# sina-behnam/RTSDS

Hardware: AMD Instinct MI355X
Metric: images/sec/node (train step) + inference FPS@1024x512, BiSeNet 19-cls (higher is better)
Workload: dtype bf16; 1 GPU; configs[1]: BiSeNet-R18 seg-only train step (train.py:65-113); model=BiSeNet-ResNet18, global_batch=8, per_gpu_batch=8, image=3x512x1024, num_classes=19, parallelism=dp1

## Files before the change

### include/rtsds_hip.h

```cpp
#ifndef RTSDS_HIP_H
#define RTSDS_HIP_H
#include <stddef.h>
#include <stdint.h>
#ifdef __cplusplus
extern "C" {
#endif

enum { RTSDS_F32 = 0, RTSDS_BF16 = 1, RTSDS_F16 = 2  };
enum {
  RTSDS_OK = 0,
  RTSDS_ERR_SHAPE = 1,
  RTSDS_ERR_UNSUPPORTED = 2,
  RTSDS_ERR_LAUNCH = 3,
  RTSDS_ERR_WORKSPACE = 4
};
enum { RTSDS_ACT_NONE = 0, RTSDS_ACT_RELU = 1, RTSDS_ACT_LEAKY = 2, RTSDS_ACT_SIGMOID = 3 };
#define RTSDS_ACCUMULATE 0x100
#define RTSDS_INPUT_PADDED 0x400
#define RTSDS_WEIGHT_PACKED 0x800

typedef struct {
  int n, h, w, c;
  int ho, wo, k;
  int kh, kw;
// ... 39 lines not shown
  int nv;
  int cv, cp;
  int splits, accumulate;
} rtsds_split_reduce_desc;
int rtsds_conv2d_wgrad_deferred(const rtsds_conv_desc* d, const void* x, const void* dy, float* dw,
                                float* dbias, int accumulate, void* ws, size_t ws_bytes,
                                rtsds_split_reduce_desc* pending, void* stream);
int rtsds_split_reduce_many(int n, const rtsds_split_reduce_desc* descs, void* stream);
size_t rtsds_imgconv_bn_wgrad_workspace(const rtsds_conv_desc* d);
int rtsds_imgconv_bn_wgrad(const rtsds_conv_desc* d, const void* x, const void* bn_dy, const void* bn_x,
                           const float* coef, int act, float* dw, int accumulate, void* ws, size_t ws_bytes,
                           void* stream);
int rtsds_imgconv_bn_wgrad_deferred(const rtsds_conv_desc* d, const void* x, const void* bn_dy, const void* bn_x,
                                    const float* coef, int act, float* dw, int accumulate, void* ws,
                                    size_t ws_bytes, rtsds_split_reduce_desc* pending, void* stream);

size_t rtsds_bn_workspace(long rows, int c);
int rtsds_bn_fwd(const void* x, const void* res, void* y, long rows, int c, const float* gamma,
                 const float* beta, float* running_mean, float* running_var,
                 long long* num_batches_tracked, float* save_mean,
                 float* save_invstd, float momentum, float eps, int training, int act,
                 const float* stats_part, int stats_nrb, int dtype, void* ws, size_t ws_bytes,
                 void* stream);
int rtsds_bn_fwd_ld(const void* x, const void* res, void* y, long ldy, long rows, int c,
                    const float* gamma, const float* beta, float* running_mean, float* running_var,
                    long long* num_batches_tracked, float* save_mean, float* save_invstd,
                    float momentum, float eps, int training, int act, const float* stats_part,
                    int stats_nrb, int dtype, void* ws, size_t ws_bytes, void* stream);
int rtsds_bn_fold(const float* gamma, const float* beta, const float* running_mean,
                  const float* running_var, const float* conv_bias, float eps, int c, float* scale,
// ... 268 lines not shown
                        void* pooled, void* hid, void* att, void* r, int ldr, int n, long hw, int c, int dtype,
                        void* stream);
int rtsds_ffm_att_bwd(const void* dr, const void* f, const void* a, const void* h, const void* p, const void* w1,
                      const void* w2, float* dw1, float* db1, float* dw2, float* db2, void* dp, int n, long hw, int c,
                      int accumulate, int dtype, void* ws, size_t ws_bytes, void* stream);
int rtsds_bn_bwd_ffm(const void* dr, const void* att, const void* dpooled, int n, long hw, const void* x, void* dx,
                     float* dgamma, float* dbeta, int c, const float* gamma, const float* beta, const float* save_mean,
                     const float* save_invstd, int training, int act, int accumulate_params, int dtype, void* ws,
                     size_t ws_bytes, void* stream);

size_t rtsds_label_stats_workspace(int n, int c);
int rtsds_label_stats(const int64_t* label, int n, int h, int w, int c, int ignore_index,
                      unsigned long long* count, unsigned long long* support, void* ws, size_t ws_bytes,
                      void* stream);

#define RTSDS_ABI_VERSION 27
int rtsds_abi_version(void);

#ifdef __cplusplus
}
#endif
#endif
```

### rtsds_amd/_lib.py

```python
import ctypes
import os

import torch

_HERE = os.path.dirname(os.path.abspath(__file__))
DEFAULT_LIB_PATH = os.path.join(_HERE, "librtsds_hip.so")
ABI_VERSION = 27
LIB_PATH = os.environ.get("RTSDS_LIB") or DEFAULT_LIB_PATH

F32, BF16 = 0, 1
ACT_NONE, ACT_RELU, ACT_LEAKY, ACT_SIGMOID = 0, 1, 2, 3
ACCUMULATE = 0x100
INPUT_PADDED = 0x400
WEIGHT_PACKED = 0x800
UPCE_SET_CORRECT = 2
ERRORS = {1: "bad shape", 2: "unsupported configuration", 3: "HIP launch failure", 4: "workspace too small"}

c_int, c_long, c_float, c_double, c_size_t, c_void_p = (ctypes.c_int, ctypes.c_long, ctypes.c_float, ctypes.c_double,
                                                        ctypes.c_size_t, ctypes.c_void_p)


class ConvDesc(ctypes.Structure):
    _fields_ = [(n, c_int) for n in ("n", "h", "w", "c", "ho", "wo", "k", "kh", "kw", "sh", "sw",
                                     "ph", "pw", "dh", "dw", "dtype")]


class SplitReduceDesc(ctypes.Structure):
    _fields_ = [("slab", c_void_p), ("dw", c_void_p), ("slab_stride", c_long), ("nv", c_int), ("cv", c_int),
                ("cp", c_int), ("splits", c_int), ("accumulate", c_int)]


class BnParams(ctypes.Structure):
    _fields_ = [("gamma", c_void_p), ("beta", c_void_p), ("running_mean", c_void_p), ("running_var", c_void_p),
                ("num_batches_tracked", c_void_p), ("save_mean", c_void_p), ("save_invstd", c_void_p),
                ("momentum", c_float), ("eps", c_float), ("stats_part", c_void_p), ("stats_nrb", c_int),
                ("accumulate", c_int), ("dgamma", c_void_p), ("dbeta", c_void_p)]


P = c_void_p
SIGNATURES = {
    "rtsds_conv2d_fwd_workspace": (c_size_t, [ctypes.POINTER(ConvDesc)]),
    "rtsds_conv2d_input_pitch": (c_int, [ctypes.POINTER(ConvDesc)]),
    "rtsds_conv2d_fwd_stats_tiles": (c_int, [ctypes.POINTER(ConvDesc)]),
    "rtsds_conv2d_fwd": (c_int, [ctypes.POINTER(ConvDesc), P, P, P, P, c_int, P, P, c_size_t, P]),
# ... 5 lines not shown
    "rtsds_conv2d_dgrad_pack_bytes": (c_size_t, [ctypes.POINTER(ConvDesc)]),
    "rtsds_conv2d_dgrad_pack_many": (c_int, [c_int, ctypes.POINTER(ConvDesc), P, P, P]),
    "rtsds_conv2d_dgrad": (c_int, [ctypes.POINTER(ConvDesc), P, P, P, c_int, P, c_size_t, P]),
    "rtsds_conv2d_dgrad_act": (c_int, [ctypes.POINTER(ConvDesc), P, P, P, P, c_int, P, c_size_t, P]),
    "rtsds_conv2d_dgrad_bnstats_tiles": (c_int, [ctypes.POINTER(ConvDesc)]),
    "rtsds_conv2d_dgrad_bnstats": (c_int, [ctypes.POINTER(ConvDesc), P, P, P, P, P, P, P, P, c_int, P, P, c_size_t, P]),
    "rtsds_conv2d_wgrad_workspace": (c_size_t, [ctypes.POINTER(ConvDesc)]),
    "rtsds_conv2d_wgrad": (c_int, [ctypes.POINTER(ConvDesc), P, P, P, P, c_int, P, c_size_t, P]),
    "rtsds_conv2d_wgrad_deferred": (c_int, [ctypes.POINTER(ConvDesc), P, P, P, P, c_int, P, c_size_t,
                                            ctypes.POINTER(SplitReduceDesc), P]),
    "rtsds_split_reduce_many": (c_int, [c_int, ctypes.POINTER(SplitReduceDesc), P]),
    "rtsds_imgconv_bn_wgrad_workspace": (c_size_t, [ctypes.POINTER(ConvDesc)]),
    "rtsds_imgconv_bn_wgrad": (c_int, [ctypes.POINTER(ConvDesc), P, P, P, P, c_int, P, c_int, P, c_size_t, P]),
    "rtsds_imgconv_bn_wgrad_deferred": (c_int, [ctypes.POINTER(ConvDesc), P, P, P, P, c_int, P, c_int, P, c_size_t,
                                                ctypes.POINTER(SplitReduceDesc), P]),
    "rtsds_bn_workspace": (c_size_t, [c_long, c_int]),
    "rtsds_bn_bwd_coef": (c_int, [P, P, P, P, P, c_long, c_int, P, P, P, P, c_int, c_int, c_int, c_int, P, c_size_t, P]),
    "rtsds_bn_fwd": (c_int, [P, P, P, c_long, c_int, P, P, P, P, P, P, P, c_float, c_float, c_int,
                             c_int, P, c_int, c_int, P, c_size_t, P]),
    "rtsds_bn_fwd_ld": (c_int, [P, P, P, c_long, c_long, c_int, P, P, P, P, P, P, P, c_float, c_float, c_int,
                                c_int, P, c_int, c_int, P, c_size_t, P]),
    "rtsds_bn_fold": (c_int, [P, P, P, P, P, c_float, c_int, P, P, P]),
    "rtsds_pooled_mlp_fwd": (c_int, [P, P, P, P, P, P, P, c_int, c_int, c_int, c_int, c_int, P]),
    "rtsds_pooled_mlp_bwd": (c_int, [P, P, P, P, P, P, P, P, P, P, P, c_int, c_int, c_int, c_int, c_int, c_int, P]),
    "rtsds_bn_fwd_gap": (c_int, [P, P, P, c_int, c_long, c_int, P, P, P, P, P, P, P, c_float, c_float, c_int, P, c_int,
                                 c_int, P, c_size_t, P]),
    "rtsds_ffm_att_scale": (c_int, [P] * 10 + [c_int, c_int, c_long, c_int, c_int, P]),
    "rtsds_ffm_att_bwd": (c_int, [P] * 12 + [c_int, c_long, c_int, c_int, c_int, P, c_size_t, P]),
    "rtsds_bn_bwd_ffm": (c_int, [P, P, P, c_int, c_long, P, P, P, P, c_int, P, P, P, P, c_int, c_int, c_int, c_int,
                                 P, c_size_t, P]),
# ... 161 lines not shown
```

### rtsds_amd/csrc/bn.hip

```cpp
#include "bn_dev.h"
#include "chan_dev.h"
#include <type_traits>
#include <algorithm>

static const int kBnMaxRB = 2048;
static const int kBnTinyRows = 64;

template <int VEC> struct BnLayout {
  int tpr, rpi;
  __host__ __device__ BnLayout(int c) {
    tpr = (c + VEC - 1) / VEC;
    if (tpr > 256) tpr = 256;
    rpi = 256 / tpr;
  }
};
template <int VEC> struct BnTile : BnLayout<VEC> {
  int cl, cv, rg, ch0, cvalid;
  bool col, active;
  RT_DEV static int block_channels(int c) { return min(c - (int)blockIdx.y * 256 * VEC, 256 * VEC); }
  RT_DEV BnTile(int c) : BnLayout<VEC>(block_channels(c)) {
    cl = block_channels(c);
    cv = threadIdx.x % this->tpr;
    rg = threadIdx.x / this->tpr;
    ch0 = blockIdx.y * 256 * VEC + cv * VEC;
    cvalid = c - ch0;
    col = cv * VEC < cl;
    active = rg < this->rpi && col;
  }
  RT_DEV long row0() const { return (long)blockIdx.x * this->rpi + rg; }
  RT_DEV long step() const { return (long)gridDim.x * this->rpi; }
};

RT_DEV void bn_coef(float g, float b, float m, float inv, float& sc, float& sh) {
  sc = g * inv;
  sh = fmaf(-m, sc, b);
}

RT_DEV void chan_merge(float& na, float& ma, float& Ma, float nb, float mb, float Mb) {
  if (nb == 0.f) return;
  if (na == 0.f) { na = nb; ma = mb; Ma = Mb; return; }
  const float n = na + nb, d = mb - ma;
  ma += d * (nb / n);
  Ma += Mb + d * d * (na * nb / n);
  na = n;
}

template <typename T, int VEC>
__global__ void __launch_bounds__(256) bn_stats_kernel(const T* __restrict__ x, float* __restrict__ part, long rows, int c) {
  __shared__ float sh[3][256][VEC];
  const BnTile<VEC> t(c);
  const int tid = threadIdx.x, ch0 = t.ch0;
// ... 436 lines not shown
  __syncthreads();
  if (t.rg != 0 || !t.col) return false;
#pragma unroll
  for (int j = 0; j < VEC; ++j) {
    float a = red[0][tid][j], b = red[1][tid][j];
    for (int gi = 1; gi < t.rpi; ++gi) {
      a += red[0][gi * t.tpr + t.cv][j];
      b += red[1][gi * t.tpr + t.cv][j];
    }
    sg[j] = a;
    sgx[j] = b;
  }
  return true;
}

struct BnBwdOps {
  float inv = 0.f, g = 1.f, bt = 0.f, mu = 0.f, dg0 = 0.f, db0 = 0.f;
};
RT_DEV BnBwdOps bn_bwd_ops(int ch, const float* gamma, const float* beta, const float* smean, const float* sinv,
                           const float* dgamma, const float* dbeta, int accumulate) {
  BnBwdOps o;
  o.inv = sinv[ch];
  o.mu = smean[ch];
  if (gamma) o.g = gamma[ch];
  if (beta) o.bt = beta[ch];
  if (accumulate && dgamma) o.dg0 = dgamma[ch];
  if (accumulate && dbeta) o.db0 = dbeta[ch];
  return o;
}
RT_DEV void bn_bwd_tail(const BnBwdOps& o, float sg, float sgx, int ch, long rows, int training, int accumulate,
                        float* dgamma, float* dbeta, float& A, float& B, float& C) {
  const float inv = o.inv;
  if (dgamma) dgamma[ch] = accumulate ? o.dg0 + sgx * inv : sgx * inv;
  if (dbeta) dbeta[ch] = accumulate ? o.db0 + sg : sg;
  const float a = o.g * inv;
  const float invn = 1.f / (float)rows;
  A = a;
  B = training ? -a * inv * inv * sgx * invn : 0.f;
  C = training ? -a * sg * invn : 0.f;
}
RT_DEV void bn_bwd_coef_rows(const BnBwdOps& o, float sg, float sgx, int ch, int c, long rows, int training, int accumulate,
                             float* dgamma, float* dbeta, float* coef) {
  bn_bwd_tail(o, sg, sgx, ch, rows, training, accumulate, dgamma, dbeta, coef[ch], coef[c + ch], coef[2 * c + ch]);
  coef[3 * c + ch] = o.mu;
  bn_coef(o.g, o.bt, o.mu, o.inv, coef[4 * c + ch], coef[5 * c + ch]);
}

template <typename T, int VEC>
RT_DEV void bn_bwd_row_store(T* __restrict__ dx, T* __restrict__ dres, long off, const BnDx<VEC>& k, int cvalid, const float* g,
                             float* xv) {
#pragma unroll
  for (int j = 0; j < VEC; ++j) xv[j] = bn_bwd_dx<VEC>(k, j, g[j], xv[j]);
  if (dx) store_vec<T, VEC>(dx + off, xv, cvalid);
  if (dres) store_vec<T, VEC>(dres + off, g, cvalid);
}
// ... 872 lines not shown
```

### rtsds_amd/csrc/bn_dev.h

```cpp
#pragma once
#include "common.h"

template <typename T, int VEC>
RT_DEV void load_vec(const T* p, float* v, int cvalid) {
  static_assert(VEC == 1 || VEC == VecT<T>::N, "VEC");
  if constexpr (VEC == VecT<T>::N) {
    typename VecT<T>::v16 t = *(const typename VecT<T>::v16*)p;
#pragma unroll
    for (int j = 0; j < VEC; ++j) v[j] = to_f(t[j]);
  } else {
    v[0] = cvalid > 0 ? to_f(p[0]) : 0.f;
  }
}
template <typename T, int VEC>
RT_DEV void store_vec(T* p, const float* v, int cvalid) {
  if constexpr (VEC == VecT<T>::N) {
    typename VecT<T>::v16 t;
#pragma unroll
    for (int j = 0; j < VEC; ++j) t[j] = from_f<T>(v[j]);
    *(typename VecT<T>::v16*)p = t;
  } else {
    if (cvalid > 0) p[0] = from_f<T>(v[0]);
  }
}

RT_DEV float act_grad(float y, int act) {
  if (act == RTSDS_ACT_RELU) return y > 0.f ? 1.f : 0.f;
  if (act == RTSDS_ACT_LEAKY) return y > 0.f ? 1.f : 0.2f;
  if (act == RTSDS_ACT_SIGMOID) return y * (1.f - y);
  return 1.f;
}

template <int VEC, bool HAS_Y>
RT_DEV void bn_mask(float* g, const float* yv, const float* xv, const float* sc, const float* sh, int act) {
  if (!act) return;
#pragma unroll
  for (int j = 0; j < VEC; ++j) {
    if constexpr (HAS_Y) g[j] *= act_grad(yv[j], act);
    else g[j] = fmaf(xv[j], sc[j], sh[j]) > 0.f ? g[j] : (act == RTSDS_ACT_LEAKY ? 0.2f * g[j] : 0.f);
  }
}

template <typename T, int VEC>
RT_DEV unsigned bn_y_bits(const float* v) {
  static_assert(VEC <= 8, "one byte per channel vector");
// ... 13 lines not shown
};

template <typename T, int VEC>
RT_DEV void bn_row_mask(float* g, const T* __restrict__ y, const float* xv, const BnDx<VEC>& k, int act, int cvalid) {
  if (!act) return;
  if (y) {
    float yv[VEC];
    load_vec<T, VEC>(y, yv, cvalid);
    bn_mask<VEC, true>(g, yv, xv, k.sc, k.sh, act);
  } else {
    bn_mask<VEC, false>(g, nullptr, xv, k.sc, k.sh, act);
  }
}
template <int VEC>
RT_DEV float bn_bwd_dx(const BnDx<VEC>& k, int j, float g, float x) { return fmaf(k.a[j], g, fmaf(k.b[j], x - k.mu[j], k.k[j])); }
```

### rtsds_amd/csrc/imgconv.hip

```cpp
#include "conv_host.h"
#include "bn_dev.h"

template <int N> RT_DEV void wait_vmcnt_img() { asm volatile("s_waitcnt vmcnt(%0)" ::"n"(N) : "memory"); }
RT_DEV float row16_sum(float v) {
  v += __builtin_bit_cast(float, __builtin_amdgcn_mov_dpp(__builtin_bit_cast(int, v), 0xB1, 0xF, 0xF, false));
  v += __builtin_bit_cast(float, __builtin_amdgcn_mov_dpp(__builtin_bit_cast(int, v), 0x4E, 0xF, 0xF, false));
  v += __builtin_bit_cast(float, __builtin_amdgcn_mov_dpp(__builtin_bit_cast(int, v), 0x141, 0xF, 0xF, false));
  v += __builtin_bit_cast(float, __builtin_amdgcn_mov_dpp(__builtin_bit_cast(int, v), 0x140, 0xF, 0xF, false));
  return v;
}
RT_DEV void store8(rsrc_t r, bf16x4 v, int off) {
#if defined(__HIP_DEVICE_COMPILE__)
  typedef __attribute__((ext_vector_type(2))) unsigned u32x2;
  __builtin_amdgcn_raw_buffer_store_b64(__builtin_bit_cast(u32x2, v), r, off, 0, 0);
#endif
}

template <int ACT>
RT_DEV float img_act(float t, int act) {
  const int a = ACT >= 0 ? ACT : act;
  if (a == RTSDS_ACT_RELU) return fmaxf(t, 0.f);
  if (a == RTSDS_ACT_LEAKY) return t > 0.f ? t : 0.2f * t;
  if (a == RTSDS_ACT_SIGMOID) return 1.f / (1.f + expf(-t));
  return t;
// ... 764 lines not shown
  }
  return rtsds_split_reduce_many(1, &q, stream);
}
extern "C" int rtsds_imgconv_bn_wgrad(const rtsds_conv_desc* d, const void* x, const void* bn_dy, const void* bn_x,
                                      const float* coef, int act, float* dw, int accumulate, void* ws, size_t ws_bytes,
                                      void* stream) {
  return img_wg_impl(d, x, bn_dy, bn_x, coef, act, dw, accumulate, ws, ws_bytes, nullptr, stream);
}
extern "C" int rtsds_imgconv_bn_wgrad_deferred(const rtsds_conv_desc* d, const void* x, const void* bn_dy, const void* bn_x,
                                               const float* coef, int act, float* dw, int accumulate, void* ws,
                                               size_t ws_bytes, rtsds_split_reduce_desc* pending, void* stream) {
  if (!pending) return RTSDS_ERR_SHAPE;
  pending->nv = 0;
  return img_wg_impl(d, x, bn_dy, bn_x, coef, act, dw, accumulate, ws, ws_bytes, pending, stream);
}
```

### rtsds_amd/functional.py

```python
import ctypes

import numpy as np
import torch

from ._lib import (ACT_RELU, ACT_SIGMOID, INPUT_PADDED, UPCE_SET_CORRECT, WEIGHT_PACKED, BnParams, ConvDesc,
                   SplitReduceDesc, lib)
from .runtime import (CL, bump_params_epoch, collective, dcode, dp_world, empty_nhwc, nhwc, params_epoch,
                      register_fold, require_hip, side_enabled, side_fork, stream, workspace)

_P = lambda t: None if t is None else t.data_ptr()

CONV_PROFILE = None


def _conv_flops(d):
    return 2.0 * d.n * d.ho * d.wo * d.k * d.c * d.kh * d.kw


class _Timed:
    def __init__(self, d, tag="fwd"):
        self.d, self.tag = d, tag

    def __enter__(self):
        if CONV_PROFILE is not None:
# ... 124 lines not shown


def _join_add(join, g):
    if join is None:
        return g
    if join.buf is not None:
        if join.first:
            join.buf.add_(g)
            return join.put(join.buf)
        g.add_(join.buf)
    return join.put(g)


DEFER_WGRAD_REDUCE = True
_deferred = []


def flush_wgrad_reduce():
    global _deferred
    items, _deferred = _deferred, []
    if not items:
        return
    cur = torch.cuda.current_stream(items[0][1].device)
    for st in {it[2] for it in items}:
        if st != cur:
            cur.wait_stream(st)
    batch, seen = [], set()
    for desc, _ws, _st in items + [(None, None, None)]:
        if desc is None or desc.dw in seen or len(batch) == 16:
            if batch:
                arr = (SplitReduceDesc * len(batch))(*batch)
                lib.rtsds_split_reduce_many(len(batch), arr, cur.cuda_stream)
            batch, seen = [], set()
        if desc is not None:
            batch.append(desc)
            seen.add(desc.dw)
    for _desc, ws, st in items:
        if st != cur:
            ws.record_stream(cur)


def _wgrad_into_arena(d, x, g, sinks, xflag, ws):
    if DEFER_WGRAD_REDUCE and CONV_PROFILE is None and x.dtype == torch.bfloat16:
        pend = SplitReduceDesc()
        lib.rtsds_conv2d_wgrad_deferred(ctypes.byref(d), _P(x), _P(g), _P(sinks[0]), _P(sinks[1]), 1 | xflag,
                                        _P(ws), ws.numel(), ctypes.byref(pend), stream())
        if pend.nv > 0:
            _deferred.append((pend, ws, torch.cuda.current_stream(ws.device)))
            torch.autograd.Variable._execution_engine.queue_callback(flush_wgrad_reduce)
        return
    with _Timed(d, "wgrad"):
# ... 21 lines not shown
        ctx.xflag = flag
        ctx.in_act, ctx.out_folded = fold
        ctx.bn_link = bn_link if join is None and not fold[0] else None
        if ctx.in_act and join is not None:
            raise RuntimeError("rtsds_amd: a conv whose input gradient is masked cannot join other readers")
        ctx.d, ctx.act, ctx.has_bias = d, act, bias is not None
        ctx.params = (weight, bias)
        ctx.wg_link = None
        if wg_link is not None:
            wg_link.conv_ok = bool(
                IMG_WGRAD_LINK and not ctx.needs_input_grad[0] and ctx.needs_input_grad[1] and bias is None and not act
                and not fold[0] and not fold[1]
                and lib.rtsds_imgconv_bn_wgrad_workspace(ctypes.byref(d)) > 0)
            if wg_link.conv_ok:
                ctx.wg_link = wg_link
        ctx.join = join
        ctx.save_for_backward(x, wq, y if act else None)
        return y

    @staticmethod
    def backward(ctx, dy):
        x, wq, y = ctx.saved_tensors
        d = ctx.d
        dy = nhwc(dy)
        if dy.dtype != x.dtype:
            dy = cast(dy, x.dtype)
        link = ctx.wg_link
        if link is not None and link.bn is not None:
            (bx, coef, bact), link.bn = link.bn, None
            return (None, _img_bn_wgrad(d, x, dy, bx, coef, bact, ctx.params[0], ctx.xflag)) + (None,) * 11
        if ctx.act and not ctx.out_folded:
            g = torch.empty_like(dy)
            lib.rtsds_act_bwd(_P(dy), _P(y), _P(g), dy.numel(), ctx.act, 1.0, dcode(dy), stream())
        else:
            g = dy
        dx = dw = db = None
        wg_side = None
        if ctx.needs_input_grad[1] and side_enabled(d.n * d.ho * d.wo) and CONV_PROFILE is None:
            weight, bias = ctx.params
            sinks = _sinks(weight, bias if ctx.needs_input_grad[2] else None)
            if sinks is not None:
                ws = workspace(lib.rtsds_conv2d_wgrad_workspace(ctypes.byref(d)), x.device)
# ... 52 lines not shown
    if sinks is not None and DEFER_WGRAD_REDUCE and CONV_PROFILE is None:
        pend = SplitReduceDesc()
        lib.rtsds_imgconv_bn_wgrad_deferred(ctypes.byref(d), _P(x), _P(g), _P(bx), _P(coef), act, _P(sinks[0]),
                                            1 | xflag, _P(ws), ws.numel(), ctypes.byref(pend), stream())
        _deferred.append((pend, ws, torch.cuda.current_stream(ws.device)))
        torch.autograd.Variable._execution_engine.queue_callback(flush_wgrad_reduce)
        return None
    dw = sinks[0] if sinks is not None else torch.empty((d.k, d.c, d.kh, d.kw), dtype=torch.float32,
                                                         device=x.device, memory_format=CL)
    with _Timed(d, "wgrad"):
        lib.rtsds_imgconv_bn_wgrad(ctypes.byref(d), _P(x), _P(g), _P(bx), _P(coef), act, _P(dw),
                                   (1 if sinks is not None else 0) | xflag, _P(ws), ws.numel(), stream())
    return None if sinks is not None else dw


def conv2d(x, weight, bias, wq, stride=(1, 1), padding=(0, 0), dilation=(1, 1), act=0, bn_stats=False,
           join=None, in_act=0, fold_out=False, bn_link=None, wg_link=None):
    stats = nrb = None
    if bn_stats and act == 0:
        n, _, h, w = x.shape
        k, _, kh, kw = weight.shape
        d = _conv_desc(x, k, kh, kw, stride, padding, dilation)
        nrb = lib.rtsds_conv2d_fwd_stats_tiles(ctypes.byref(d))
        stats = torch.empty(nrb * k * 4, dtype=torch.float32, device=x.device)
    y = ConvFn.apply(x, weight, bias, wq, tuple(stride), tuple(padding), tuple(dilation), act, stats, join,
                     (in_act, bool(fold_out and act in (1, 2))), bn_link, wg_link)
    if stats is not None:
        y._rt_bn_stats = (stats, nrb)
    return y

# ... 147 lines not shown

BN_BWD_LINK = True


class BnBwdLink:

    __slots__ = ("src", "part", "nrb")

    def __init__(self):
        self.src = None
        self.part = None
        self.nrb = 0


IMG_WGRAD_LINK = True


class ImgWgradLink:

    __slots__ = ("conv_ok", "bn")

    def __init__(self):
        self.conv_ok = False
        self.bn = None

    def take(self, x, training, act):
        if IMG_WGRAD_LINK and self.conv_ok and training and act in (0, 1, 2) and x.dtype == torch.bfloat16 \
                and not getattr(x, "_backward_hooks", None):
            return self
        return None


def _bn_bwd_coef(ctx_link, dy, x, dg, db, rows, c, gamma, beta, sm, si, training, act, acc):
    coef = torch.empty(6 * c, dtype=torch.float32, device=x.device)
    ws = workspace(lib.rtsds_bn_workspace(rows, c), x.device)
    lib.rtsds_bn_bwd_coef(_P(dy), _P(x), _P(dg), _P(db), _P(coef), rows, c, _P(gamma), _P(beta), _P(sm), _P(si),
                          training, act, acc, dcode(x), _P(ws), ws.numel(), stream())
    ctx_link.bn = (x, coef, act)


RES_BN_PAIR = True
RES_BN_BITS = False


def _res_bits_ok(x, res, training, act):
    return (training and res is not None and act == ACT_RELU and x.shape[1] % 8 == 0
            and x.dtype in (torch.bfloat16, torch.float32) and res.dtype == x.dtype and res.shape == x.shape)

# ... 1632 lines not shown
```

Measured before the change: 1887 images/s.

## Fuse BN backward stats into stem image-conv wgrad as one-pass kernel

Adds a one-pass kernel for the image-input stem conv that reads the BN output gradient and BN input once. It applies the ReLU mask, accumulates the BN sum(g) and sum(g*(x-mu)) via extra MFMAs against a ones vector and against x, and computes the weight gradient of g in the same sweep. A combine kernel then derives dgamma/dbeta and applies the BN linear correction to dw analytically. This replaces the separate BN coef reduction pass over the large stem activation. In exchange it doubles the MFMA work and adds split-reduce plus combine launches, and it depends on the BN correction being folded exactly.

```diff
diff --git a/include/rtsds_hip.h b/include/rtsds_hip.h
--- a/include/rtsds_hip.h
+++ b/include/rtsds_hip.h
@@ -77,6 +77,28 @@
 int rtsds_imgconv_bn_wgrad_deferred(const rtsds_conv_desc* d, const void* x, const void* bn_dy, const void* bn_x,
                                     const float* coef, int act, float* dw, int accumulate, void* ws,
                                     size_t ws_bytes, rtsds_split_reduce_desc* pending, void* stream);
+typedef struct {
+  const float* sums;
+  const float* slab;
+  long slab_stride;
+  int splits;
+  const float *gamma, *beta, *mean, *invstd;
+  float *dgamma, *dbeta, *dw;
+  long rows;
+  int k3;
+  int accumulate_bn, accumulate_dw;
+} rtsds_imgconv_bn_combine_desc;
+size_t rtsds_imgconv_bn_onepass_workspace(const rtsds_conv_desc* d);
+int rtsds_imgconv_bn_onepass(const rtsds_conv_desc* d, const void* x, const void* bn_dy, const void* bn_x,
+                             const float* gamma, const float* beta, const float* mean, const float* invstd, int act,
+                             float* dgamma, float* dbeta, int accumulate_bn, float* dw, int accumulate, void* ws,
+                             size_t ws_bytes, void* stream);
+int rtsds_imgconv_bn_onepass_deferred(const rtsds_conv_desc* d, const void* x, const void* bn_dy, const void* bn_x,
+                                      const float* gamma, const float* beta, const float* mean, const float* invstd,
+                                      int act, float* dgamma, float* dbeta, int accumulate_bn, float* dw, int accumulate,
+                                      void* ws, size_t ws_bytes, rtsds_split_reduce_desc* pending,
+                                      rtsds_imgconv_bn_combine_desc* combine, void* stream);
+int rtsds_imgconv_bn_combine(const rtsds_imgconv_bn_combine_desc* c, void* stream);
 
 size_t rtsds_bn_workspace(long rows, int c);
 int rtsds_bn_fwd(const void* x, const void* res, void* y, long rows, int c, const float* gamma,
@@ -375,7 +397,7 @@
                       unsigned long long* count, unsigned long long* support, void* ws, size_t ws_bytes,
                       void* stream);
 
-#define RTSDS_ABI_VERSION 27
+#define RTSDS_ABI_VERSION 28
 int rtsds_abi_version(void);
 
 #ifdef __cplusplus
diff --git a/rtsds_amd/_lib.py b/rtsds_amd/_lib.py
--- a/rtsds_amd/_lib.py
+++ b/rtsds_amd/_lib.py
@@ -5,7 +5,7 @@
 
 _HERE = os.path.dirname(os.path.abspath(__file__))
 DEFAULT_LIB_PATH = os.path.join(_HERE, "librtsds_hip.so")
-ABI_VERSION = 27
+ABI_VERSION = 28
 LIB_PATH = os.environ.get("RTSDS_LIB") or DEFAULT_LIB_PATH
 
 F32, BF16 = 0, 1
@@ -28,6 +28,12 @@
 class SplitReduceDesc(ctypes.Structure):
     _fields_ = [("slab", c_void_p), ("dw", c_void_p), ("slab_stride", c_long), ("nv", c_int), ("cv", c_int),
                 ("cp", c_int), ("splits", c_int), ("accumulate", c_int)]
+
+
+class ImgBnCombineDesc(ctypes.Structure):
+    _fields_ = [("sums", c_void_p), ("slab", c_void_p), ("slab_stride", c_long), ("splits", c_int), ("gamma", c_void_p), ("beta", c_void_p), ("mean", c_void_p), ("invstd", c_void_p),
+                ("dgamma", c_void_p), ("dbeta", c_void_p), ("dw", c_void_p), ("rows", c_long), ("k3", c_int),
+                ("accumulate_bn", c_int), ("accumulate_dw", c_int)]
 
 
 class BnParams(ctypes.Structure):
@@ -63,6 +69,13 @@
     "rtsds_imgconv_bn_wgrad": (c_int, [ctypes.POINTER(ConvDesc), P, P, P, P, c_int, P, c_int, P, c_size_t, P]),
     "rtsds_imgconv_bn_wgrad_deferred": (c_int, [ctypes.POINTER(ConvDesc), P, P, P, P, c_int, P, c_int, P, c_size_t,
                                                 ctypes.POINTER(SplitReduceDesc), P]),
+    "rtsds_imgconv_bn_onepass_workspace": (c_size_t, [ctypes.POINTER(ConvDesc)]),
+    "rtsds_imgconv_bn_onepass": (c_int, [ctypes.POINTER(ConvDesc), P, P, P, P, P, P, P, c_int, P, P, c_int, P, c_int, P,
+                                         c_size_t, P]),
+    "rtsds_imgconv_bn_onepass_deferred": (c_int, [ctypes.POINTER(ConvDesc), P, P, P, P, P, P, P, c_int, P, P, c_int, P,
+                                                  c_int, P, c_size_t, ctypes.POINTER(SplitReduceDesc),
+                                                  ctypes.POINTER(ImgBnCombineDesc), P]),
+    "rtsds_imgconv_bn_combine": (c_int, [ctypes.POINTER(ImgBnCombineDesc), P]),
     "rtsds_bn_workspace": (c_size_t, [c_long, c_int]),
     "rtsds_bn_bwd_coef": (c_int, [P, P, P, P, P, c_long, c_int, P, P, P, P, c_int, c_int, c_int, c_int, P, c_size_t, P]),
     "rtsds_bn_fwd": (c_int, [P, P, P, c_long, c_int, P, P, P, P, P, P, P, c_float, c_float, c_int,
diff --git a/rtsds_amd/csrc/bn.hip b/rtsds_amd/csrc/bn.hip
--- a/rtsds_amd/csrc/bn.hip
+++ b/rtsds_amd/csrc/bn.hip
@@ -30,11 +30,6 @@
   RT_DEV long row0() const { return (long)blockIdx.x * this->rpi + rg; }
   RT_DEV long step() const { return (long)gridDim.x * this->rpi; }
 };
-
-RT_DEV void bn_coef(float g, float b, float m, float inv, float& sc, float& sh) {
-  sc = g * inv;
-  sh = fmaf(-m, sc, b);
-}
 
 RT_DEV void chan_merge(float& na, float& ma, float& Ma, float nb, float mb, float Mb) {
   if (nb == 0.f) return;
@@ -501,31 +496,6 @@
   return true;
 }
 
-struct BnBwdOps {
-  float inv = 0.f, g = 1.f, bt = 0.f, mu = 0.f, dg0 = 0.f, db0 = 0.f;
-};
-RT_DEV BnBwdOps bn_bwd_ops(int ch, const float* gamma, const float* beta, const float* smean, const float* sinv,
-                           const float* dgamma, const float* dbeta, int accumulate) {
-  BnBwdOps o;
-  o.inv = sinv[ch];
-  o.mu = smean[ch];
-  if (gamma) o.g = gamma[ch];
-  if (beta) o.bt = beta[ch];
-  if (accumulate && dgamma) o.dg0 = dgamma[ch];
-  if (accumulate && dbeta) o.db0 = dbeta[ch];
-  return o;
-}
-RT_DEV void bn_bwd_tail(const BnBwdOps& o, float sg, float sgx, int ch, long rows, int training, int accumulate,
-                        float* dgamma, float* dbeta, float& A, float& B, float& C) {
-  const float inv = o.inv;
-  if (dgamma) dgamma[ch] = accumulate ? o.dg0 + sgx * inv : sgx * inv;
-  if (dbeta) dbeta[ch] = accumulate ? o.db0 + sg : sg;
-  const float a = o.g * inv;
-  const float invn = 1.f / (float)rows;
-  A = a;
-  B = training ? -a * inv * inv * sgx * invn : 0.f;
-  C = training ? -a * sg * invn : 0.f;
-}
 RT_DEV void bn_bwd_coef_rows(const BnBwdOps& o, float sg, float sgx, int ch, int c, long rows, int training, int accumulate,
                              float* dgamma, float* dbeta, float* coef) {
   bn_bwd_tail(o, sg, sgx, ch, rows, training, accumulate, dgamma, dbeta, coef[ch], coef[c + ch], coef[2 * c + ch]);
diff --git a/rtsds_amd/csrc/bn_dev.h b/rtsds_amd/csrc/bn_dev.h
--- a/rtsds_amd/csrc/bn_dev.h
+++ b/rtsds_amd/csrc/bn_dev.h
@@ -29,6 +29,11 @@
   if (act == RTSDS_ACT_LEAKY) return y > 0.f ? 1.f : 0.2f;
   if (act == RTSDS_ACT_SIGMOID) return y * (1.f - y);
   return 1.f;
+}
+
+RT_DEV void bn_coef(float g, float b, float m, float inv, float& sc, float& sh) {
+  sc = g * inv;
+  sh = fmaf(-m, sc, b);
 }
 
 template <int VEC, bool HAS_Y>
@@ -72,3 +77,29 @@
 }
 template <int VEC>
 RT_DEV float bn_bwd_dx(const BnDx<VEC>& k, int j, float g, float x) { return fmaf(k.a[j], g, fmaf(k.b[j], x - k.mu[j], k.k[j])); }
+
+struct BnBwdOps {
+  float inv = 0.f, g = 1.f, bt = 0.f, mu = 0.f, dg0 = 0.f, db0 = 0.f;
+};
+RT_DEV BnBwdOps bn_bwd_ops(int ch, const float* gamma, const float* beta, const float* smean, const float* sinv,
+                           const float* dgamma, const float* dbeta, int accumulate) {
+  BnBwdOps o;
+  o.inv = sinv[ch];
+  o.mu = smean[ch];
+  if (gamma) o.g = gamma[ch];
+  if (beta) o.bt = beta[ch];
+  if (accumulate && dgamma) o.dg0 = dgamma[ch];
+  if (accumulate && dbeta) o.db0 = dbeta[ch];
+  return o;
+}
+RT_DEV void bn_bwd_tail(const BnBwdOps& o, float sg, float sgx, int ch, long rows, int training, int accumulate,
+                        float* dgamma, float* dbeta, float& A, float& B, float& C) {
+  const float inv = o.inv;
+  if (dgamma) dgamma[ch] = accumulate ? o.dg0 + sgx * inv : sgx * inv;
+  if (dbeta) dbeta[ch] = accumulate ? o.db0 + sg : sg;
+  const float a = o.g * inv;
+  const float invn = 1.f / (float)rows;
+  A = a;
+  B = training ? -a * inv * inv * sgx * invn : 0.f;
+  C = training ? -a * sg * invn : 0.f;
+}
diff --git a/rtsds_amd/csrc/imgconv.hip b/rtsds_amd/csrc/imgconv.hip
--- a/rtsds_amd/csrc/imgconv.hip
+++ b/rtsds_amd/csrc/imgconv.hip
@@ -802,3 +802,394 @@
   pending->nv = 0;
   return img_wg_impl(d, x, bn_dy, bn_x, coef, act, dw, accumulate, ws, ws_bytes, pending, stream);
 }
+
+struct ImgOpArgs {
+  const bf16* x4;
+  const bf16* g;
+  const bf16* xb;
+  const float *gamma, *beta, *mean, *invstd;
+  float* slab;
+  int stride;
+  int n, h, w, ho, wo, ph, pw;
+  int tiles, per;
+};
+static int img_op_stride(int kh, int kw) { return (129 * kh * kw * 3 + 2 * kCo + 3) & ~3; }
+
+template <int KH, int KW, int NT, int WN, int ACT>
+__global__ void __launch_bounds__(NT, NT == 256 ? 2 : 1) imgconv_bn_onepass_kernel(const ImgOpArgs P) {
+  static_assert(ACT == RTSDS_ACT_NONE || ACT == RTSDS_ACT_RELU, "masked g must stay an exact bf16");
+  constexpr int KWP = (KW + 1) / 2, NJ = KWP / 2, NB = KH * NJ;
+  constexpr int NW = NT / 64;
+  static_assert(KWP % 2 == 0 && NB % WN == 0 && NW % WN == 0 && 4 % (NW / WN) == 0, "wave layout");
+  constexpr int WM = NW / WN, CB = 4 / WM, NBW = NB / WN, NPB = (NBW + WM - 1) / WM;
+  constexpr int NR = 2 * kTH + KH - 2, NC = kTW + KWP - 1, NP = NR * NC;
+  constexpr int NI = (NP + 63) / 64, NIW = (NI + NW - 1) / NW, A_BYTES = NI * 1024;
+  constexpr int HP = kTH * kTW / 2;
+  constexpr int T_BYTES = HP * kCo * 2;
+  constexpr int K3 = KH * KW * 3;
+  constexpr int PQ = NT / 8, U = HP / PQ;
+  __shared__ __attribute__((aligned(16))) float cf[3 * kCo];
+  __shared__ __attribute__((aligned(16))) float red[NW][kCo][2];
+  __shared__ __attribute__((aligned(16))) unsigned char gts[T_BYTES];
+  __shared__ __attribute__((aligned(16))) unsigned char xts[T_BYTES];
+  __shared__ __attribute__((aligned(16))) unsigned char ones[HP * 8];
+  __shared__ __attribute__((aligned(16))) unsigned char abuf0[A_BYTES];
+  __shared__ __attribute__((aligned(16))) unsigned char abuf1[A_BYTES];
+
+  const int tid = threadIdx.x, lane = tid & 63, wave = __builtin_amdgcn_readfirstlane(tid >> 6);
+  int bid;
+  {
+    const int nwg = gridDim.x, b = blockIdx.x;
+    const int xcd = b & 7, q = nwg >> 3, r = nwg & 7;
+    bid = (xcd < r ? xcd * (q + 1) : r * (q + 1) + (xcd - r) * q) + (b >> 3);
+  }
+  const int t0 = bid * P.per, t1 = min(P.tiles, t0 + P.per);
+  const int tw_n = (P.wo + kTW - 1) / kTW, th_n = (P.ho + kTH - 1) / kTH;
+  const int spw = P.w >> 1, pwp = (P.pw + 1) >> 1;
+  const int ybytes = P.n * P.ho * P.wo * kCo * 2;
+  const rsrc_t rx = make_rsrc(P.x4, P.n * P.h * P.w * 8);
+  const rsrc_t rg = make_rsrc(P.g, ybytes), rb = make_rsrc(P.xb, ybytes);
+  auto tile_xy = [&](int t, int& img, int& oh0, int& ow0) {
+    img = t / (th_n * tw_n);
+    const int rem = t - img * th_n * tw_n, trow = rem / tw_n;
+    oh0 = trow * kTH;
+    ow0 = (rem - trow * tw_n) * kTW;
+  };
+  auto issue = [&](int t, unsigned char* dst) {
+    int img, oh0, ow0;
+    tile_xy(t, img, oh0, ow0);
+    const int ih0 = 2 * oh0 - P.ph, j0 = ow0 - pwp;
+#pragma unroll
+    for (int i = 0; i < NIW; ++i) {
+      const int ins = wave + NW * i;
+      if (ins < NI) {
+        const int piece = ins * 64 + lane;
+        const int row = piece / NC, col = piece - row * NC;
+        const int ih = ih0 + row, j = j0 + col;
+        const bool ok = piece < NP && (unsigned)ih < (unsigned)P.h && (unsigned)j < (unsigned)spw;
+        buf_lds16(rx, dst + ins * 1024, ok ? ((img * P.h + ih) * spw + j) * 16 : (int)0x80000000, 0);
+      }
+    }
+  };
+  const int cg = tid & 7, pq = tid >> 3;
+  u32x4_img gv[U], xv[U];
+  auto fetch = [&](int t, int hh) {
+    int img, oh0, ow0;
+    tile_xy(t, img, oh0, ow0);
+#pragma unroll
+    for (int u = 0; u < U; ++u) {
+      const int px = pq + PQ * u, oh = oh0 + 2 * hh + (px >> 6), ow = ow0 + (px & 63);
+      const int off = (oh < P.ho && ow < P.wo) ? (((img * P.ho + oh) * P.wo + ow) * kCo + 8 * cg) * 2 : (int)0x80000000;
+      gv[u] = img_load16(rg, off);
+      xv[u] = img_load16(rb, off);
+    }
+  };
+
+  if (tid < kCo) {
+    const float mu = P.mean[tid];
+    float sc, sh;
+    bn_coef(P.gamma ? P.gamma[tid] : 1.f, P.beta ? P.beta[tid] : 0.f, mu, P.invstd[tid], sc, sh);
+    cf[tid] = mu;
+    cf[kCo + tid] = sc;
+    cf[2 * kCo + tid] = sh;
+  }
+  issue(t0, abuf0);
+  fetch(t0, 0);
+
+  const int g4 = lane >> 4, L = 4 * g4 + ((lane >> 2) & 3), p8 = (lane & 3) * 8;
+  const int wm = wave / WN, wn = wave % WN;
+  const int aoff = L * 16 + p8;
+  int doff[CB];
+#pragma unroll
+  for (int cb = 0; cb < CB; ++cb) doff[cb] = L * 128 + (((wm * CB + cb) ^ ((L >> 1) & 3)) << 5) + p8;
+  const unsigned char* const obase = ones + L * 8;
+  f32x4 acc[2 * CB][NBW], pacc[NPB];
+#pragma unroll
+  for (int cb = 0; cb < 2 * CB; ++cb)
+#pragma unroll
+    for (int j = 0; j < NBW; ++j) acc[cb][j] = f32x4{0.f, 0.f, 0.f, 0.f};
+#pragma unroll
+  for (int j = 0; j < NPB; ++j) pacc[j] = f32x4{0.f, 0.f, 0.f, 0.f};
+  float sg[8], sgx[8];
+#pragma unroll
+  for (int j = 0; j < 8; ++j) sg[j] = sgx[j] = 0.f;
+
+  auto half = [&](int t, auto bc, auto hc) {
+    constexpr int B = decltype(bc)::value, HH = decltype(hc)::value;
+    int img, oh0, ow0;
+    tile_xy(t, img, oh0, ow0);
+    asm volatile("s_waitcnt vmcnt(0)" ::: "memory");
+    __syncthreads();
+    {
+      BnDx<8> k;
+#pragma unroll
+      for (int q = 0; q < 2; ++q) {
+        const f32x4 vm = *(const f32x4*)(cf + 8 * cg + 4 * q), vs = *(const f32x4*)(cf + kCo + 8 * cg + 4 * q);
+        const f32x4 vh = *(const f32x4*)(cf + 2 * kCo + 8 * cg + 4 * q);
+#pragma unroll
+        for (int e = 0; e < 4; ++e) { k.mu[4 * q + e] = vm[e]; k.sc[4 * q + e] = vs[e]; k.sh[4 * q + e] = vh[e]; }
+      }
+#pragma unroll
+      for (int u = 0; u < U; ++u) {
+        const int px = pq + PQ * u;
+        const bool ok = oh0 + 2 * HH + (px >> 6) < P.ho && ow0 + (px & 63) < P.wo;
+        const bf16x8 gb = __builtin_bit_cast(bf16x8, gv[u]), xb = __builtin_bit_cast(bf16x8, xv[u]);
+        float gf[8], xf[8];
+#pragma unroll
+        for (int j = 0; j < 8; ++j) { gf[j] = to_f(gb[j]); xf[j] = to_f(xb[j]); }
+        bn_row_mask<bf16, 8>(gf, (const bf16*)nullptr, xf, k, ACT, 8);
+        bf16x8 o;
+#pragma unroll
+        for (int j = 0; j < 8; ++j) {
+          sg[j] += gf[j];
+          sgx[j] = fmaf(gf[j], xf[j] - k.mu[j], sgx[j]);
+          o[j] = from_f<bf16>(gf[j]);
+        }
+        const int so = px * 128 + ((((cg >> 1) ^ ((px >> 1) & 3))) << 5) + (cg & 1) * 16;
+        *(bf16x8*)(gts + so) = o;
+        *(u32x4_img*)(xts + so) = xv[u];
+        const bf16 one = ok ? (bf16)1.f : (bf16)0.f;
+        *(bf16x4*)(ones + px * 8) = bf16x4{one, one, one, one};
+        __builtin_amdgcn_sched_barrier(0);
+      }
+    }
+    __syncthreads();
+    if (HH == 0) {
+      if (t + 1 < t1) issue(t + 1, B ? abuf0 : abuf1);
+      fetch(t, 1);
+    } else if (t + 1 < t1) {
+      fetch(t + 1, 0);
+    }
+    const unsigned char* ab = (B ? abuf1 : abuf0) + aoff;
+#pragma unroll
+    for (int kl = 0; kl < kTH; ++kl) {
+      bf16x8 fd[2 * CB], fa[NBW];
+#pragma unroll
+      for (int cb = 0; cb < CB; ++cb) {
+        fd[cb] = img_tr_frag(gts + doff[cb] + 32 * kl * 128, gts + doff[cb] + (32 * kl + 16) * 128);
+        fd[CB + cb] = img_tr_frag(xts + doff[cb] + 32 * kl * 128, xts + doff[cb] + (32 * kl + 16) * 128);
+      }
+      const bf16x8 f1 = img_tr_frag(obase + 32 * kl * 8, obase + (32 * kl + 16) * 8);
+#pragma unroll
+      for (int j = 0; j < NBW; ++j) {
+        const int nb = wn * NBW + j, r = nb / NJ, jj = nb - r * NJ;
+        const unsigned char* a0 = ab + ((2 * (2 * HH + (kl >> 1)) + r) * NC + 32 * (kl & 1) + 2 * jj) * 16;
+        fa[j] = img_tr_frag(a0, a0 + 256);
+      }
+#pragma unroll
+      for (int cb = 0; cb < 2 * CB; ++cb)
+#pragma unroll
+        for (int j = 0; j < NBW; ++j) acc[cb][j] = __builtin_amdgcn_mfma_f32_16x16x32_bf16(fa[j], fd[cb], acc[cb][j], 0, 0, 0);
+#pragma unroll
+      for (int j = 0; j < NBW; ++j)
+        if (j % WM == wm) pacc[j / WM] = __builtin_amdgcn_mfma_f32_16x16x32_bf16(fa[j], f1, pacc[j / WM], 0, 0, 0);
+      __builtin_amdgcn_sched_barrier(0);
+    }
+  };
+  for (int t = t0; t < t1; t += 2) {
+    half(t, std::integral_constant<int, 0>(), std::integral_constant<int, 0>());
+    half(t, std::integral_constant<int, 0>(), std::integral_constant<int, 1>());
+    if (t + 1 < t1) {
+      half(t + 1, std::integral_constant<int, 1>(), std::integral_constant<int, 0>());
+      half(t + 1, std::integral_constant<int, 1>(), std::integral_constant<int, 1>());
+    }
+  }
+  float* out = P.slab + (long)bid * P.stride;
+#pragma unroll
+  for (int j = 0; j < NBW; ++j) {
+    const int nb = wn * NBW + j, r = nb / NJ, jj = nb - r * NJ;
+    const int s = 2 * (2 * jj + (g4 >> 1)) - 1 + (g4 & 1);
+    if (s >= 0 && s < KW) {
+      const int tap = (r * KW + s) * 3;
+#pragma unroll
+      for (int cb = 0; cb < 2 * CB; ++cb) {
+        const int row = (cb < CB ? 0 : kCo) + 16 * (wm * CB + cb % CB) + (lane & 15);
+        float* o = out + row * K3 + tap;
+        o[0] = acc[cb][j][0];
+        o[1] = acc[cb][j][1];
+        o[2] = acc[cb][j][2];
+      }
+      if (j % WM == wm && (lane & 15) == 0) {
+        float* o = out + 2 * kCo * K3 + tap;
+        o[0] = pacc[j / WM][0];
+        o[1] = pacc[j / WM][1];
+        o[2] = pacc[j / WM][2];
+      }
+    }
+  }
+#pragma unroll
+  for (int o = 8; o < 64; o <<= 1)
+#pragma unroll
+    for (int j = 0; j < 8; ++j) {
+      sg[j] += __shfl_xor(sg[j], o, 64);
+      sgx[j] += __shfl_xor(sgx[j], o, 64);
+    }
+  if (lane < 8) {
+#pragma unroll
+    for (int j = 0; j < 8; ++j) { red[wave][8 * lane + j][0] = sg[j]; red[wave][8 * lane + j][1] = sgx[j]; }
+  }
+  __syncthreads();
+  if (tid < 2 * kCo) {
+    const int ch = tid >> 1, w = tid & 1;
+    float s = red[0][ch][w];
+#pragma unroll
+    for (int v = 1; v < NW; ++v) s += red[v][ch][w];
+    out[129 * K3 + tid] = s;
+  }
+  for (int i = 129 * K3 + 2 * kCo + tid; i < P.stride; i += NT) out[i] = 0.f;
+}
+
+struct ImgCombArgs {
+  const float* p;
+  const float* slab;
+  long stride;
+  int splits;
+  const float *gamma, *beta, *mean, *invstd;
+  float *dgamma, *dbeta, *dw;
+  long rows;
+  int k3, acc_bn, acc_dw;
+};
+__global__ void __launch_bounds__(256) imgconv_bn_combine_kernel(const ImgCombArgs a) {
+  const int co = blockIdx.x, k3 = a.k3;
+  const BnBwdOps ops = bn_bwd_ops(co, a.gamma, a.beta, a.mean, a.invstd, a.dgamma, a.dbeta, a.acc_bn);
+  __shared__ double rd[2][256];
+  {
+    double s0 = 0.0, s1 = 0.0;
+    for (int w = threadIdx.x; w < a.splits; w += 256) {
+      const float* q = a.slab + (long)w * a.stride + 129 * k3 + 2 * co;
+      s0 += (double)q[0];
+      s1 += (double)q[1];
+    }
+    rd[0][threadIdx.x] = s0;
+    rd[1][threadIdx.x] = s1;
+    __syncthreads();
+    for (int s = 128; s > 0; s >>= 1) {
+      if ((int)threadIdx.x < s) {
+        rd[0][threadIdx.x] += rd[0][threadIdx.x + s];
+        rd[1][threadIdx.x] += rd[1][threadIdx.x + s];
+      }
+      __syncthreads();
+    }
+  }
+  const float sg = (float)rd[0][0], sgx = (float)rd[1][0];
+  float A, B, C, dgv, dbv;
+  bn_bwd_tail(ops, sg, sgx, 0, a.rows, 1, 0, &dgv, &dbv, A, B, C);
+  asm volatile("" : "+v"(dgv));
+  if (threadIdx.x == 0) {
+    if (a.dgamma) a.dgamma[co] = a.acc_bn ? __fadd_rn(ops.dg0, dgv) : dgv;
+    if (a.dbeta) a.dbeta[co] = a.acc_bn ? __fadd_rn(ops.db0, dbv) : dbv;
+  }
+  for (int i = threadIdx.x; i < k3; i += 256) {
+    const float p1 = a.p[co * k3 + i], p2 = a.p[(kCo + co) * k3 + i], p3 = a.p[2 * kCo * k3 + i];
+    const float v = fmaf(A, p1, fmaf(B, p2 - ops.mu * p3, C * p3));
+    float* o = a.dw + co * k3 + i;
+    *o = a.acc_dw ? __fadd_rn(*o, v) : v;
+  }
+}
+
+template <int ACT>
+static const void* img_op_kernel_act(int kh) {
+  return kh == 7 ? (const void*)imgconv_bn_onepass_kernel<7, 7, 512, 2, ACT> : (const void*)imgconv_bn_onepass_kernel<3, 3, 256, 1, ACT>;
+}
+static int img_op_threads(int kh) { return kh == 7 ? 512 : 256; }
+static const void* img_op_kernel(int kh, int act) {
+  return act == RTSDS_ACT_RELU ? img_op_kernel_act<RTSDS_ACT_RELU>(kh) : img_op_kernel_act<RTSDS_ACT_NONE>(kh);
+}
+static void img_op_grid(const rtsds_conv_desc* d, int& grid, int& per) {
+  static int occ[2] = {0, 0}, cus = 0;
+  const int v = d->kh == 7;
+  if (!occ[v] && (hipOccupancyMaxActiveBlocksPerMultiprocessor(&occ[v], img_op_kernel(d->kh, RTSDS_ACT_RELU), img_op_threads(d->kh), 0) != hipSuccess ||
+                  occ[v] < 1))
+    occ[v] = 1;
+  if (!cus && (hipDeviceGetAttribute(&cus, hipDeviceAttributeMultiprocessorCount, 0) != hipSuccess || cus < 1)) cus = 256;
+  const int tiles = img_tiles(d), slots = cus * occ[v];
+  per = (tiles + slots - 1) / slots;
+  grid = (tiles + per - 1) / per;
+}
+static size_t img_op_slab_bytes(const rtsds_conv_desc* d) {
+  int grid, per;
+  img_op_grid(d, grid, per);
+  return al256((size_t)grid * img_op_stride(d->kh, d->kw) * 4);
+}
+static size_t img_op_sum_bytes(const rtsds_conv_desc* d) { return al256((size_t)img_op_stride(d->kh, d->kw) * 4); }
+extern "C" size_t rtsds_imgconv_bn_onepass_workspace(const rtsds_conv_desc* d) {
+  return img_wg_ok(d) ? img_op_slab_bytes(d) + img_op_sum_bytes(d) + sp_x4_bytes(d) : 0;
+}
+extern "C" int rtsds_imgconv_bn_combine(const rtsds_imgconv_bn_combine_desc* c, void* stream) {
+  if (!c || !c->sums || !c->slab || c->splits <= 0 || !c->mean || !c->invstd || !c->dw || c->k3 <= 0 || c->rows <= 0) return RTSDS_ERR_SHAPE;
+  ImgCombArgs a;
+  a.p = c->sums; a.slab = c->slab; a.stride = c->slab_stride; a.splits = c->splits; a.gamma = c->gamma; a.beta = c->beta; a.mean = c->mean; a.invstd = c->invstd;
+  a.dgamma = c->dgamma; a.dbeta = c->dbeta; a.dw = c->dw; a.rows = c->rows; a.k3 = c->k3;
+  a.acc_bn = c->accumulate_bn ? 1 : 0; a.acc_dw = c->accumulate_dw ? 1 : 0;
+  hipLaunchKernelGGL(imgconv_bn_combine_kernel, dim3(kCo), dim3(256), 0, (hipStream_t)stream, a);
+  RET_LAUNCH();
+}
+static int img_op_impl(const rtsds_conv_desc* d, const void* x, const void* bn_dy, const void* bn_x, const float* gamma,
+                       const float* beta, const float* mean, const float* invstd, int act, float* dgamma, float* dbeta,
+                       int accumulate_bn, float* dw, int accumulate, void* ws, size_t ws_bytes,
+                       rtsds_split_reduce_desc* pending, rtsds_imgconv_bn_combine_desc* combine, void* stream) {
+  if (!img_wg_ok(d)) return check_desc(d) ? check_desc(d) : RTSDS_ERR_UNSUPPORTED;
+  if (!(act == RTSDS_ACT_NONE || act == RTSDS_ACT_RELU)) return RTSDS_ERR_UNSUPPORTED;
+  if (!x || !bn_dy || !bn_x || !mean || !invstd || !dw) return RTSDS_ERR_SHAPE;
+  const bool x_padded = (accumulate & RTSDS_INPUT_PADDED) != 0;
+  accumulate &= ~RTSDS_INPUT_PADDED;
+  if (ws_bytes < rtsds_imgconv_bn_onepass_workspace(d)) return RTSDS_ERR_WORKSPACE;
+  hipStream_t st = (hipStream_t)stream;
+  const size_t slab_bytes = img_op_slab_bytes(d), sum_bytes = img_op_sum_bytes(d);
+  float* sums = (float*)((char*)ws + slab_bytes);
+  if (!x_padded) {
+    void* x4 = (char*)ws + slab_bytes + sum_bytes;
+    sp_pad4(d, x, x4, st);
+    x = x4;
+  }
+  ImgOpArgs a;
+  a.x4 = (const bf16*)x; a.g = (const bf16*)bn_dy; a.xb = (const bf16*)bn_x;
+  a.gamma = gamma; a.beta = beta; a.mean = mean; a.invstd = invstd; a.slab = (float*)ws;
+  a.stride = img_op_stride(d->kh, d->kw);
+  a.n = d->n; a.h = d->h; a.w = d->w; a.ho = d->ho; a.wo = d->wo; a.ph = d->ph; a.pw = d->pw;
+  a.tiles = img_tiles(d);
+  int grid;
+  img_op_grid(d, grid, a.per);
+  void* args[] = {&a};
+  (void)hipLaunchKernel(img_op_kernel(d->kh, act), dim3(grid), dim3(img_op_threads(d->kh)), args, 0, st);
+  rtsds_split_reduce_desc q;
+  q.slab = (const float*)ws;
+  q.dw = sums;
+  q.slab_stride = a.stride;
+  q.nv = a.stride / 4;
+  q.cv = 1;
+  q.cp = 4;
+  q.splits = grid;
+  q.accumulate = 0;
+  rtsds_imgconv_bn_combine_desc c;
+  c.sums = sums; c.slab = (const float*)ws; c.slab_stride = a.stride; c.splits = grid; c.gamma = gamma; c.beta = beta; c.mean = mean; c.invstd = invstd;
+  c.dgamma = dgamma; c.dbeta = dbeta; c.dw = dw;
+  c.rows = (long)d->n * d->ho * d->wo;
+  c.k3 = d->kh * d->kw * 3;
+  c.accumulate_bn = accumulate_bn ? 1 : 0;
+  c.accumulate_dw = accumulate ? 1 : 0;
+  if (pending) {
+    *pending = q;
+    *combine = c;
+    RET_LAUNCH();
+  }
+  const int rc = rtsds_split_reduce_many(1, &q, stream);
+  return rc ? rc : rtsds_imgconv_bn_combine(&c, stream);
+}
+extern "C" int rtsds_imgconv_bn_onepass(const rtsds_conv_desc* d, const void* x, const void* bn_dy, const void* bn_x,
+                                        const float* gamma, const float* beta, const float* mean, const float* invstd, int act,
+                                        float* dgamma, float* dbeta, int accumulate_bn, float* dw, int accumulate, void* ws,
+                                        size_t ws_bytes, void* stream) {
+  return img_op_impl(d, x, bn_dy, bn_x, gamma, beta, mean, invstd, act, dgamma, dbeta, accumulate_bn, dw, accumulate, ws,
+                     ws_bytes, nullptr, nullptr, stream);
+}
+extern "C" int rtsds_imgconv_bn_onepass_deferred(const rtsds_conv_desc* d, const void* x, const void* bn_dy, const void* bn_x,
+                                                 const float* gamma, const float* beta, const float* mean, const float* invstd,
+                                                 int act, float* dgamma, float* dbeta, int accumulate_bn, float* dw,
+                                                 int accumulate, void* ws, size_t ws_bytes, rtsds_split_reduce_desc* pending,
+                                                 rtsds_imgconv_bn_combine_desc* combine, void* stream) {
+  if (!pending || !combine) return RTSDS_ERR_SHAPE;
+  pending->nv = 0;
+  return img_op_impl(d, x, bn_dy, bn_x, gamma, beta, mean, invstd, act, dgamma, dbeta, accumulate_bn, dw, accumulate, ws,
+                     ws_bytes, pending, combine, stream);
+}
diff --git a/rtsds_amd/functional.py b/rtsds_amd/functional.py
--- a/rtsds_amd/functional.py
+++ b/rtsds_amd/functional.py
@@ -4,7 +4,7 @@
 import torch
 
 from ._lib import (ACT_RELU, ACT_SIGMOID, INPUT_PADDED, UPCE_SET_CORRECT, WEIGHT_PACKED, BnParams, ConvDesc,
-                   SplitReduceDesc, lib)
+                   ImgBnCombineDesc, SplitReduceDesc, lib)
 from .runtime import (CL, bump_params_epoch, collective, dcode, dp_world, empty_nhwc, nhwc, params_epoch,
                       register_fold, require_hip, side_enabled, side_fork, stream, workspace)
 
@@ -162,11 +162,13 @@
 
 DEFER_WGRAD_REDUCE = True
 _deferred = []
+_combines = []
 
 
 def flush_wgrad_reduce():
-    global _deferred
+    global _deferred, _combines
     items, _deferred = _deferred, []
+    combines, _combines = _combines, []
     if not items:
         return
     cur = torch.cuda.current_stream(items[0][1].device)
@@ -183,6 +185,8 @@
         if desc is not None:
             batch.append(desc)
             seen.add(desc.dw)
+    for comb, _keep in combines:
+        lib.rtsds_imgconv_bn_combine(ctypes.byref(comb), cur.cuda_stream)
     for _desc, ws, st in items:
         if st != cur:
             ws.record_stream(cur)
@@ -234,6 +238,8 @@
                 and lib.rtsds_imgconv_bn_wgrad_workspace(ctypes.byref(d)) > 0)
             if wg_link.conv_ok:
                 ctx.wg_link = wg_link
+                wg_link.conv = (weight, kh, d.n * d.ho * d.wo,
+                                lib.rtsds_imgconv_bn_onepass_workspace(ctypes.byref(d)) > 0)
         ctx.join = join
         ctx.save_for_backward(x, wq, y if act else None)
         return y
@@ -246,6 +252,10 @@
         if dy.dtype != x.dtype:
             dy = cast(dy, x.dtype)
         link = ctx.wg_link
+        if link is not None and link.one is not None:
+            one, link.one = link.one, None
+            _img_bn_onepass(d, x, dy, one, ctx.params[0], ctx.xflag)
+            return (None,) * 13
         if link is not None and link.bn is not None:
             (bx, coef, bact), link.bn = link.bn, None
             return (None, _img_bn_wgrad(d, x, dy, bx, coef, bact, ctx.params[0], ctx.xflag)) + (None,) * 11
@@ -328,6 +338,24 @@
     return None if sinks is not None else dw
 
 
+def _img_bn_onepass(d, x, g, one, weight, xflag):
+    bx, gamma, beta, sm, si, dg, db, act = one
+    ws = workspace(lib.rtsds_imgconv_bn_onepass_workspace(ctypes.byref(d)), x.device)
+    dw = _sink(weight)
+    if DEFER_WGRAD_REDUCE and CONV_PROFILE is None:
+        pend, comb = SplitReduceDesc(), ImgBnCombineDesc()
+        lib.rtsds_imgconv_bn_onepass_deferred(ctypes.byref(d), _P(x), _P(g), _P(bx), _P(gamma), _P(beta), _P(sm), _P(si),
+                                              act, _P(dg), _P(db), 1, _P(dw), 1 | xflag, _P(ws), ws.numel(),
+                                              ctypes.byref(pend), ctypes.byref(comb), stream())
+        _deferred.append((pend, ws, torch.cuda.current_stream(ws.device)))
+        _combines.append((comb, one))
+        torch.autograd.Variable._execution_engine.queue_callback(flush_wgrad_reduce)
+        return
+    with _Timed(d, "wgrad"):
+        lib.rtsds_imgconv_bn_onepass(ctypes.byref(d), _P(x), _P(g), _P(bx), _P(gamma), _P(beta), _P(sm), _P(si), act,
+                                     _P(dg), _P(db), 1, _P(dw), 1 | xflag, _P(ws), ws.numel(), stream())
+
+
 def conv2d(x, weight, bias, wq, stride=(1, 1), padding=(0, 0), dilation=(1, 1), act=0, bn_stats=False,
            join=None, in_act=0, fold_out=False, bn_link=None, wg_link=None):
     stats = nrb = None
@@ -505,15 +533,20 @@
 
 
 IMG_WGRAD_LINK = True
+IMG_BN_ONEPASS = True
+IMG_BN_ONEPASS_KH = (3, 7)
+IMG_BN_ONEPASS_MIN_ROWS = 32768
 
 
 class ImgWgradLink:
 
-    __slots__ = ("conv_ok", "bn")
+    __slots__ = ("conv_ok", "bn", "conv", "one")
 
     def __init__(self):
         self.conv_ok = False
         self.bn = None
+        self.conv = None
+        self.one = None
 
     def take(self, x, training, act):
         if IMG_WGRAD_LINK and self.conv_ok and training and act in (0, 1, 2) and x.dtype == torch.bfloat16 \
@@ -523,6 +556,13 @@
 
 
 def _bn_bwd_coef(ctx_link, dy, x, dg, db, rows, c, gamma, beta, sm, si, training, act, acc):
+    conv = ctx_link.conv
+    if IMG_BN_ONEPASS and conv is not None and conv[3] and conv[1] in IMG_BN_ONEPASS_KH and training \
+            and act in (0, ACT_RELU) and x.dtype == torch.bfloat16 and dy.dtype == torch.bfloat16 \
+            and rows == conv[2] and rows >= IMG_BN_ONEPASS_MIN_ROWS and acc and dg is not None and db is not None \
+            and _sink(conv[0]) is not None:
+        ctx_link.one = (x, gamma, beta, sm, si, dg, db, act)
+        return
     coef = torch.empty(6 * c, dtype=torch.float32, device=x.device)
     ws = workspace(lib.rtsds_bn_workspace(rows, c), x.device)
     lib.rtsds_bn_bwd_coef(_P(dy), _P(x), _P(dg), _P(db), _P(coef), rows, c, _P(gamma), _P(beta), _P(sm), _P(si),
```

Measured after the change: 1897 images/s (median of 6 runs). Within noise of the previous version (+0.6%).
